# COMBINE-lab/RapMap

Measured on AMD Instinct MI355X. Metric: Mreads/s (paired 2x100 bp; one unit = one read pair), higher is better.
Workload: dtype u8/int32/u64 (integer & byte work, no floating point)

## Files before the change

### rapmap_amd/csrc/qm_host.hip

```cpp
#include <fcntl.h>
#include <hip/hip_runtime.h>
#include <sys/mman.h>
#include <sys/stat.h>
#include <unistd.h>

#include <atomic>
#include <cmath>
#include <cstdarg>
#include <cstdio>
#include <cstdlib>
#include <cstring>
#include <deque>
#include <string>
#include <vector>
#include <thread>
#include <map>
#include <memory>
#include <mutex>
#include <condition_variable>
#include <functional>

#include "qm_mapper.inl"
#include "qm_lean.inl"
#include "qm_device.h"
#include "qm_phflat.h"

using namespace qm;

static thread_local char g_err[512] = "";
static int fail(int code, const char* fmt, ...) {
  va_list ap; va_start(ap, fmt); vsnprintf(g_err, sizeof(g_err), fmt, ap); va_end(ap);
  return code;
}
#define HIPCHK(x) do { hipError_t _e = (x); if (_e != hipSuccess) return fail(QM_E_NOGPU, "%s: %s", #x, hipGetErrorString(_e)); } while (0)

struct MMap {
  void* p = nullptr; size_t len = 0;
  int open(const std::string& path) {
    int fd = ::open(path.c_str(), O_RDONLY);
    if (fd < 0) return -1;
    struct stat st; if (fstat(fd, &st) != 0) { ::close(fd); return -1; }
    len = (size_t)st.st_size;
    if (len == 0) { ::close(fd); return -1; }
    p = mmap(nullptr, len, PROT_READ, MAP_PRIVATE, fd, 0);
    ::close(fd);
    if (p == MAP_FAILED) { p = nullptr; return -1; }
    return 0;
  }
  void close() { if (p) munmap(p, len); p = nullptr; }
};

struct qm_index {
  std::string dir;
  int k = 31; bool big = false, perfect = false;
  MMap sa, txp, rsd, hash;
  const uint32_t* SA = nullptr; int64_t nSA = 0;
  std::vector<std::string> names;
  const uint32_t* offsets = nullptr; int64_t nTxp = 0;
// ... 130 lines not shown
  DevBuf<long long> d_toff;
  DevBuf<qm_hit> d_tmp; DevBuf<unsigned char> d_sides; DevBuf<int> d_tsc;
  DevBuf<int> d_tref; DevBuf<u64> d_torder; DevBuf<unsigned char> d_tasks;
  DevBuf<long long> d_ivcsr, d_lcsr;
  DevBuf<qm_sa_interval_hit> d_ivC; DevBuf<u64> d_wordsC;
  PinBuf<long long> h_tot;
  LastResult last; CallStats stats;
  uint32_t flags = 0; bool isHelper = false;
  std::vector<qm_ctx*> helpers; struct SplitPool* pool = nullptr;
};

struct SplitPool {
  std::vector<std::thread> th; std::mutex mu; std::condition_variable cv, done;
  std::function<void(int)> job; unsigned long gen = 0; int pending = 0, parts = 0; bool stop = false;
  explicit SplitPool(int n) {
    for (int i = 0; i < n; ++i) th.emplace_back([this, i]() {
      unsigned long seen = 0;
      for (;;) {
        std::function<void(int)> j;
        { std::unique_lock<std::mutex> lk(mu); cv.wait(lk, [&] { return stop || (gen != seen && i < parts); }); if (stop) return; seen = gen; j = job; }
        j(i);
        { std::lock_guard<std::mutex> lk(mu); if (--pending == 0) done.notify_all(); }
      }
    });
  }
  void run(int n, std::function<void(int)> f) {
    std::unique_lock<std::mutex> lk(mu);
    job = std::move(f); parts = n; pending = n; ++gen;
    cv.notify_all();
    done.wait(lk, [&] { return pending == 0; });
  }
  ~SplitPool() { { std::lock_guard<std::mutex> lk(mu); stop = true; } cv.notify_all(); for (auto& t : th) t.join(); }
};
struct SplitJoin {
  qm_ctx* owner; int K; std::mutex mu; std::condition_variable cv;
  long long total[8] = {0}, base[9] = {0}; int arrived = 0; bool ready = false; int failed = 0;
  int arrive(int part, long long tot, long long& b, qm_hit*& dst);
  void abort(int rc) { std::lock_guard<std::mutex> lk(mu); if (!failed) failed = rc ? rc : QM_E_STATE; cv.notify_all(); }
  bool stagger = false; int turn = 0;
  int wait_turn(int part) {
    if (!stagger) return QM_OK;
    std::unique_lock<std::mutex> lk(mu);
    cv.wait(lk, [&] { return turn >= part || failed; });
    return failed ? fail(failed, "another part of the batch failed") : QM_OK;
  }
  void pass_turn(int part) { if (!stagger) return; std::lock_guard<std::mutex> lk(mu); if (turn < part + 1) turn = part + 1; cv.notify_all(); }
};

static void begin_call(qm_ctx* c) { c->last.invalidate(); c->stats = CallStats(); }

extern "C" {

const char* qm_last_error(void) { return g_err; }
const char* qm_version(void) { return "qmap_mi355 0.1 (RapMap 0.6.0 quasimap hot path, gfx950)"; }

int qm_opts_default(qm_opts* o) {
  if (!o) return fail(QM_E_ARG, "null opts");
  o->sensitive = 1; o->strict_check = 1; o->max_num_hits = 200; o->no_orphans = 0; o->no_dovetail = 0;
  o->fuzzy = 0; o->max_interval = 1000; o->sel_aln = 0; o->quasi_cov = 0.0;
  o->hard_filter = 0; o->match_score = 2; o->mismatch_penalty = -4; o->gap_open = 4; o->gap_extend = 2; o->dp_bandwidth = 15;
  o->max_mmp_extension = 7; o->aln_policy = 0; o->min_score_fraction = 0.65; o->consensus_slack = 0.2;
  return QM_OK;
}

static bool json_field(const std::string& js, const char* name, std::string& out) {
  std::string key = std::string("\"") + name + "\"";
  size_t p = js.find(key);
  if (p == std::string::npos) return false;
  p = js.find(':', p);
  if (p == std::string::npos) return false;
  ++p;
// ... 738 lines not shown

enum { QM_STAGE_RETRY = 1 };
static int stage_verdict(qm_ctx* c, const StagePlan& p, const u64* hscal) {
  const int status = (int)(hscal[QM_SC_STATUS] & 0xffffffffu); int rc;
  if (status & 4) return fail(QM_E_TOOLONG, "a read is longer than %d characters (-s: the alignment kernels are sized for that; otherwise the long-read pass takes up to %d)", QM_MAX_LONG_READ_LEN, QM_MAX_LONG_READ_LEN);
  if (status & 2) return fail(QM_E_UNSUPPORTED, "an SA-interval list exceeded %d entries (max_interval too large)", QM_GCAP);
  if (status & 8) return fail(QM_E_STATE, "selective alignment: a read overflowed the scratch sized for it (internal error)");
  if (status & 64) return fail(QM_E_STATE, "a wavefront found no free scratch slot on its XCD (internal error)");
  if (!(status & 17)) return QM_OK;
  if (status & 1) {
    int64_t want = (int64_t)hscal[0] + p.nreads + (int64_t)p.grid * 4 * QM_CHUNK;
    if (want < c->d_lists.cap * 2) want = c->d_lists.cap * 2;
    if ((rc = c->d_lists.ensure(want))) return rc;
  }
  if (status & 16) {
    int64_t want = (int64_t)hscal[QM_SC_IVCUR] + p.nreads + (int64_t)p.grid * 4 * QM_IVCHUNK;
    if (want < c->d_iv.cap * 2) want = c->d_iv.cap * 2;
    if ((rc = c->d_iv.ensure(want))) return rc;
  }
  c->stats.relaunches += 1;
  return QM_STAGE_RETRY;
}

static int run_stage_a(qm_ctx* c, const qm_opts* o, const RunReq& rq, int64_t n, const void* d_seq1, const void* d_off1, const void* d_seq2,
                       const void* d_off2, int ns, ChunkFeeder* feeder, u64* hscal) {
  int rc; StagePlan p;
  if ((rc = plan_stage_a(c, o, rq, d_seq2 != nullptr, n, ns, p))) return rc;
  if ((rc = reserve_stage_a(c, o, rq, p))) return rc;
  const DevIndex ix = dev_index(c);
  const int64_t nreads = p.nreads;
  if (lean_first(p)) c->stats.leanReads = nreads;
  if (p.first == SK_DUO) c->stats.duoPairs = n;
  float extraMs = 0;
  while (true) {
    ReadBatch B;
    fill_batch(c, o, rq, p, d_seq1, d_off1, d_seq2, d_off2, B);
    ReadBatch H = B;
    if (p.twoPass) { H.iv_in = c->d_iv; H.iv_in_off = c->d_ivoff; H.iv_in_cnt = c->d_ivcnt; H.found_in = c->d_found; H.iv_out = nullptr; H.found_out = nullptr; }
    HIPCHK(hipMemsetAsync(c->d_scal, 0, QM_SC_WORDS * sizeof(u64), c->stream));
    if (rq.mode == QM_RUN_COLLECT || p.twoPass) HIPCHK(hipMemsetAsync(c->d_lcnt, 0, (size_t)(nreads + 1) * sizeof(uint32_t), c->stream));
    HIPCHK(hipEventRecord(c->ev0, c->stream));
    if ((rc = launch_first(c, p, rq, ix, B, feeder))) return rc;
    feeder = nullptr;
    if (p.first == SK_LEAN_SEL && nreads > 0) {
      if ((rc = read_scalars(c, hscal)) || (rc = pass_n_aware(c, p, ix, B, hscal, extraMs)) || (rc = pass_lean_leftovers(c, p, ix, B, hscal, extraMs))) return rc;
      c->stats.leanReads = nreads;
    }
    if (p.twoPass && rq.longReads && nreads > 0 && ((rc = read_scalars(c, hscal)) || (rc = pass_long_reads(c, p, ix, B, hscal, -32)))) return rc;
    if ((rc = run_list_kernels(c, p, rq, ix, H))) return rc;
    HIPCHK(hipEventRecord(c->ev1, c->stream));
    if ((rc = read_scalars(c, hscal))) return rc;
    if (lean_first(p) && ((rc = pass_n_aware(c, p, ix, B, hscal, extraMs)) || (rc = pass_lean_leftovers(c, p, ix, B, hscal, extraMs)))) return rc;
    if ((!o->sel_aln || rq.mode == QM_RUN_COLLECT) && rq.mode != QM_RUN_FROM_INTERVALS && (rc = pass_long_reads(c, p, ix, B, hscal, rq.mode == QM_RUN_COLLECT ? -32 : 32))) return rc;
    if ((rc = pass_sel_slow(c, o, rq, ix, H, hscal))) return rc;
#ifdef QM_TIMING
    {
      static const char* nm[7] = {"read->LDS", "strand setup", "probe windows", "extension", "collector rest", "hits->mappings", "write-out+loop"};
      double tot = 0; for (int i = 0; i < 7; ++i) tot += (double)hscal[20 + i];
      for (int i = 0; i < 7; ++i) fprintf(stderr, "[qm timing] %-16s %6.2f %%  %10.0f clk/read\n", nm[i], 100.0 * hscal[20 + i] / tot, (double)hscal[20 + i] / (double)nreads);
      static const char* hm[8] = {"intervals in", "suffix gather", "sort", "groups+chain", "list assembly", "(after)", "write-out", "-"};
      double ht = 0; for (int i = 0; i < 8; ++i) ht += (double)hscal[32 + i];
      if (ht > 0) for (int i = 0; i < 8; ++i) fprintf(stderr, "[qm timing h2m] %-16s %6.2f %%  %10.0f clk/read\n", hm[i], 100.0 * hscal[32 + i] / ht, (double)hscal[32 + i] / (double)nreads);
      static const char* pm[8] = {"cand+intervals", "gather+keys", "rank sort", "heads+count", "chaining", "words", "write-out", "chaining, parallel"};
      double pt = 0; for (int i = 0; i < 8; ++i) pt += (double)hscal[40 + i];
      if (pt > 0) for (int i = 0; i < 8; ++i) fprintf(stderr, "[qm timing pack] %-16s %6.2f %%  %10.0f clk/read\n", pm[i], 100.0 * hscal[40 + i] / pt, (double)hscal[40 + i] / (double)nreads);
    }
#endif
    if ((rc = stage_verdict(c, p, hscal)) == QM_STAGE_RETRY) continue;
    if (rc) return rc;
    break;
  }
  c->stats.skipped = (int64_t)hscal[QM_SC_SKIPCNT];
  if (c->stats.skipped > 0) {
    c->stats.skipList.resize((size_t)(c->stats.skipped < QM_SKIP_CAP ? c->stats.skipped : QM_SKIP_CAP));
    HIPCHK(hipMemcpy(c->stats.skipList.data(), c->d_skip, c->stats.skipList.size() * sizeof(u64), hipMemcpyDeviceToHost));
  }
  if (p.wantIv) { c->last.ivTotal = (int64_t)hscal[QM_SC_IVCUR]; c->last.ivReads = nreads; }
  if (p.wantFound) c->last.foundReads = nreads;
  if (rq.mode != QM_RUN_COLLECT && !p.duoMerge) c->last.listReads = nreads;
  c->last.listWords = (int64_t)hscal[0];
  float ms = 0; hipEventElapsedTime(&ms, c->ev0, c->ev1); c->last.mapMs = ms + extraMs;
  return QM_OK;
}
// ... 69 lines not shown
      for (int i = 0; i < K; ++i) {
        Ak[i] = A; Ak[i].u0 = cu[i]; Ak[i].u1 = cu[i + 1];
        Ak[i].tasks = (SelTask*)(c->d_tasks + (size_t)(2 * cslot[i] + 2 * i) * qmk_sel_task_bytes());
        Ak[i].ntasks = c->d_ntk + i;
        Ak[i].sides = (SelSide*)(c->d_sides + (size_t)(2 * cslot[i] + 2 * i) * qmk_sel_side_bytes());
        Ak[i].nsides = c->d_ntk + QM_SEL_CHUNKS_B + i;
        Ak[i].torder = c->d_torder + (size_t)(2 * cslot[i] + 2 * i);
        if (!noStrip) { Ak[i].torder2 = c->d_torder + (size_t)(2 * slots + 2 * K + 2) + (size_t)(2 * cslot[i] + 2 * i); Ak[i].ntasks2 = c->d_ntk + 2 * QM_SEL_CHUNKS_B + i; }
        HIPCHK(qmk_sel_plan(&P, &Ak[i], c->numCU, planStream));
        if (K > 1) HIPCHK(hipEventRecord(c->evPlan[i], planStream));
      }
      for (int i = 0; i < K; ++i) {
        if (K > 1) HIPCHK(hipStreamWaitEvent(c->stream, c->evPlan[i], 0));
        HIPCHK(qmk_sel_align_finish(&P, &Ak[i], c->numCU, c->stream));
      }
    }
  } else {
    HIPCHK(qmk_pair_count(&P, c->stream));
  }
  HIPCHK(qmk_scan_counts(c->d_scanTmp, (size_t)c->d_scanTmp.cap, c->d_cnt, c->d_offs, n + 1, c->stream));
  total = 0;
  HIPCHK(hipMemcpyAsync(&total, c->d_offs + n, sizeof(long long), hipMemcpyDeviceToHost, c->stream));
  HIPCHK(hipMemcpyAsync(hscal, c->d_scal, QM_SC_WORDS * sizeof(u64), hipMemcpyDeviceToHost, c->stream));
  u64 h[3 * QM_SEL_CHUNKS_B];
  const bool selStats = o->sel_aln && !rq.mergeOnly;
  if (selStats) HIPCHK(hipMemcpyAsync(h, c->d_ntk, sizeof(h), hipMemcpyDeviceToHost, c->stream));
  HIPCHK(hipStreamSynchronize(c->stream));
  if (selStats) {
    for (int i = 0; i < QM_SEL_CHUNKS_B; ++i) { c->stats.kswTasks += (int64_t)h[i]; c->stats.selQuestions += (int64_t)h[QM_SEL_CHUNKS_B + i]; c->stats.stripTasks += (int64_t)h[2 * QM_SEL_CHUNKS_B + i]; }
    static const bool dbg = [] { const char* e = getenv("QM_SEL_DEBUG"); return e && atoi(e) != 0; }();
    if (dbg) fprintf(stderr, "[qm -s] %lld units: %lld alignment questions beyond PERFECT chains, %lld ksw2 alignments, %lld strip alignments\n", (long long)n, (long long)c->stats.selQuestions, (long long)c->stats.kswTasks, (long long)c->stats.stripTasks);
  }
  if (rq.join) {
    long long b = 0; qm_hit* dst = nullptr;
    if ((rc = rq.join->arrive(rq.part, total, b, dst))) return rc;
    P.hits = dst + b;
  } else {
    if ((rc = c->d_hits.ensure((int64_t)total + 1, total / 8))) return rc;
    P.hits = c->d_hits;
  }
  if (o->sel_aln) HIPCHK(qmk_sel_compact(&P, c->d_tmp, c->d_toff, c->stream));
  else HIPCHK(qmk_pair_write(&P, c->stream));
  return QM_OK;
}

static int map_device_impl(qm_ctx* c, const qm_opts* o, int64_t n, const void* d_seq1, const void* d_off1, const void* d_seq2,
                           const void* d_off2, int32_t max_read_len, int64_t* n_hits, qm_counters* counters, ChunkFeeder* feeder,
                           const RunReq& rq = RunReq(), int32_t short_read_len = 0) {
  if (!c || n < 0 || (n > 0 && (!d_seq1 || !d_off1))) return fail(QM_E_ARG, "bad argument");
  int rc = check_opts(o);
  if (rc) return rc;
  if ((d_seq2 == nullptr) != (d_off2 == nullptr)) return fail(QM_E_ARG, "seq2/off2 must both be given or both be null");
  HIPCHK(hipSetDevice(c->device));
  const int pick = (max_read_len > QM_MAX_READ_LEN && short_read_len > 0) ? short_read_len : (max_read_len > QM_MAX_READ_LEN ? QM_MAX_READ_LEN : max_read_len);
  const int ns = pick <= 128 ? 2 : (pick <= 192 ? 3 : (pick <= 256 ? 4 : 8));
  const bool paired = d_seq2 != nullptr;
  u64 hscal[QM_SC_WORDS];
  begin_call(c);
  HIPCHK(hipEventRecord(c->evA, c->stream));
  RunReq r2 = rq;
  r2.keepIntervals = rq.keepIntervals || c->debug != 0;
  r2.longReads = max_read_len > QM_MAX_READ_LEN;
  r2.shortLen = pick;
  if (rq.join && (rc = rq.join->wait_turn(rq.part))) return rc;
  rc = run_stage_a(c, o, r2, n, d_seq1, d_off1, d_seq2, d_off2, ns, feeder, hscal);
  if (rq.join) rq.join->pass_turn(rq.part);
  if (rc) return rc;
  if (r2.stageView) {
    const int64_t nreads = paired ? 2 * n : n;
    if ((rc = c->d_ivcsr.ensure(nreads + 1))) return rc;
    if ((rc = c->d_lcsr.ensure(nreads + 1))) return rc;
    if ((rc = c->h_tot.ensure(2))) return rc;
    if ((rc = ensure_scan_tmp(c, nreads + 1))) return rc;
    if (!r2.keepIntervals) {
      if ((rc = c->d_ivcnt.ensure(nreads + 1))) return rc;
      if ((rc = c->d_ivoff.ensure(nreads + 1))) return rc;
      if ((rc = c->d_iv.ensure(1))) return rc;
      HIPCHK(hipMemsetAsync(c->d_ivcnt, 0, (size_t)(nreads + 1) * sizeof(uint32_t), c->stream));
      HIPCHK(hipMemsetAsync(c->d_ivoff, 0, (size_t)(nreads + 1) * sizeof(long long), c->stream));
    }
    HIPCHK(hipMemsetAsync(c->d_ivcnt + nreads, 0, sizeof(uint32_t), c->stream));
    HIPCHK(hipMemsetAsync(c->d_lcnt + nreads, 0, sizeof(uint32_t), c->stream));
    HIPCHK(qmk_scan_counts(c->d_scanTmp, (size_t)c->d_scanTmp.cap, c->d_ivcnt, c->d_ivcsr, nreads + 1, c->stream));
    HIPCHK(qmk_scan_counts_masked(c->d_scanTmp, (size_t)c->d_scanTmp.cap, c->d_lcnt, c->d_lcsr, nreads + 1, c->stream));
    HIPCHK(hipMemcpyAsync(&c->h_tot[0], c->d_ivcsr + nreads, sizeof(long long), hipMemcpyDeviceToHost, c->stream));
    HIPCHK(hipMemcpyAsync(&c->h_tot[1], c->d_lcsr + nreads, sizeof(long long), hipMemcpyDeviceToHost, c->stream));
    c->last.stReads = nreads;
  }
  long long total = 0;
  if ((rc = run_stage_b(c, o, r2, n, paired, d_seq1, d_off1, d_seq2, d_off2, hscal, total))) return rc;
  HIPCHK(hipEventRecord(c->evB, c->stream));
  HIPCHK(hipStreamSynchronize(c->stream));
  float ms = 0; hipEventElapsedTime(&ms, c->evA, c->evB); c->last.totalMs = ms;
  c->last.units = n; c->last.hits = total; c->last.paired = paired;
  if (r2.stageView) c->last.stUnits = n;
  if (n_hits) *n_hits = total;
  if (counters) *counters = counters_from(hscal);
  return QM_OK;
}

int SplitJoin::arrive(int part, long long tot, long long& b, qm_hit*& dst) {
  std::unique_lock<std::mutex> lk(mu);
  total[part] = tot;
  if (++arrived == K && !failed) {
    for (int i = 0; i < K; ++i) base[i + 1] = base[i] + total[i];
    const int rc = owner->d_hits.ensure((int64_t)base[K] + 1, base[K] / 8);
    if (rc) failed = rc; else ready = true;
    cv.notify_all();
  }
  cv.wait(lk, [&] { return ready || failed; });
  if (failed) return failed == QM_E_NOMEM ? fail(QM_E_NOMEM, "hipMalloc of the result array failed") : fail(failed, "another part of the batch failed");
  b = base[part]; dst = owner->d_hits;
  return QM_OK;
}

static int map_device_split(qm_ctx* c, const qm_opts* o, int K, int64_t n, const void* d_seq1, const void* d_off1, const void* d_seq2,
                            const void* d_off2, int32_t max_read_len, int64_t* n_hits, qm_counters* counters) {
  int rc;
  HIPCHK(hipSetDevice(c->device));
  while ((int)c->helpers.size() < K) {
    qm_ctx* h = nullptr;
    if ((rc = qm_ctx_create_ex(c->ix, c->device, c->flags, &h))) return rc;
    h->isHelper = true; c->helpers.push_back(h);
  }
  if (!c->pool || (int)c->pool->th.size() < K) { delete c->pool; c->pool = new SplitPool(K); }
  if ((rc = c->d_offs.ensure(n + 1))) return rc;
  SplitJoin J; J.owner = c; J.K = K;
  { const char* sg = getenv("QM_SPLIT_STAGGER"); J.stagger = sg ? atoi(sg) != 0 : false; }
  int64_t nh[8] = {0}; qm_counters ctr[8]; int rcs[8] = {0}; char errs[8][256];
  memset(ctr, 0, sizeof(ctr));
  const bool paired = d_seq2 != nullptr;
  static const int firstPct = [] { const char* e = getenv("QM_SPLIT_FIRST"); const int v = e ? atoi(e) : 0; return v > 0 && v < 100 ? v : 0; }();
  static const int duoParts = [] { const char* e = getenv("QM_DUO_PARTS"); return e ? atoi(e) : 0x55; }();
  begin_call(c);
  HIPCHK(hipEventRecord(c->evA, c->stream));
  c->pool->run(K, [&](int i) {
    qm_ctx* h = c->helpers[(size_t)i];
    int64_t u0 = n * i / K, u1 = n * (i + 1) / K;
    if (K == 2 && firstPct > 0) { const int64_t cut = n * firstPct / 100; u0 = i == 0 ? 0 : cut; u1 = i == 0 ? cut : n; }
    RunReq rq; rq.join = &J; rq.part = i;
    rq.noDuo = ((duoParts >> i) & 1) == 0;
    errs[i][0] = 0;
    int r = map_device_impl(h, o, u1 - u0, d_seq1, (const long long*)d_off1 + u0, d_seq2, d_seq2 ? (const long long*)d_off2 + u0 : nullptr,
                            max_read_len, &nh[i], &ctr[i], nullptr, rq);
    if (r == QM_OK) {
      hipError_t e = qmk_rebase_offsets(h->d_offs, c->d_offs + u0, (u1 - u0) + (i == K - 1 ? 1 : 0), J.base[i], h->stream);
      if (e == hipSuccess) e = hipStreamSynchronize(h->stream);
      if (e != hipSuccess) r = fail(QM_E_NOGPU, "rebasing a part's offsets: %s", hipGetErrorString(e));
    }
    if (r != QM_OK) { snprintf(errs[i], sizeof(errs[i]), "%s", g_err); J.abort(r); }
    rcs[i] = r;
  });
  for (int i = 0; i < K; ++i) if (rcs[i]) return fail(rcs[i], "%s", errs[i]);
  HIPCHK(hipEventRecord(c->evB, c->stream));
  HIPCHK(hipEventSynchronize(c->evB));
  float first = 1e30f, last = 0, t = 0;
  for (int i = 0; i < K; ++i) {
    qm_ctx* h = c->helpers[(size_t)i];
    if (hipEventElapsedTime(&t, c->evA, h->ev0) == hipSuccess && t < first) first = t;
    if (hipEventElapsedTime(&t, c->evA, h->ev1) == hipSuccess && t > last) last = t;
  }
  c->last.mapMs = last > first ? last - first : 0;
  float ms = 0; hipEventElapsedTime(&ms, c->evA, c->evB); c->last.totalMs = ms;
  qm_counters sum; memset(&sum, 0, sizeof(sum));
  for (int i = 0; i < K; ++i) {
    sum += ctr[i];
    int64_t u0 = n * i / K;
    if (K == 2 && firstPct > 0) u0 = i == 0 ? 0 : n * firstPct / 100;
    c->stats.add_part(c->helpers[(size_t)i]->stats, paired ? 2 * u0 : u0);
  }
  c->last.units = n; c->last.hits = J.base[K]; c->last.paired = paired;
  if (n_hits) *n_hits = J.base[K];
  if (counters) *counters = sum;
  return QM_OK;
}

int qm_map_device(qm_ctx* c, const qm_opts* o, int64_t n, const void* d_seq1, const void* d_off1, const void* d_seq2,
                  const void* d_off2, int32_t max_read_len, int64_t* n_hits, qm_counters* counters) {
  const char* me = getenv("QM_SPLIT_MIN");
  const int64_t minUnits = me && atoll(me) > 0 ? atoll(me) : ((int64_t)1 << 21);
  if (c && o && !c->isHelper && !c->debug && n >= minUnits && d_seq1 && d_off1 && (d_seq2 == nullptr) == (d_off2 == nullptr) && check_opts(o) == QM_OK) {
    const char* se = getenv("QM_SPLIT");
    int K = se ? atoi(se) : 2;
    if (K > 8) K = 8;
    if (K > 1) return map_device_split(c, o, K, n, d_seq1, d_off1, d_seq2, d_off2, max_read_len, n_hits, counters);
  }
  return map_device_impl(c, o, n, d_seq1, d_off1, d_seq2, d_off2, max_read_len, n_hits, counters, nullptr);
}

static int stage_offsets(qm_ctx* c, int64_t n, const int64_t* off, DevBuf<uint8_t>& d_seq, DevBuf<long long>& d_off, int32_t& maxLen,
                         int32_t& maxShort) {
  for (int64_t i = 0; i < n; ++i) {
    int64_t l = off[i + 1] - off[i];
    if (l < 0) return fail(QM_E_ARG, "offsets not monotone");
    if (l > maxLen) maxLen = (int32_t)(l > 0x7fffffff ? 0x7fffffff : l);
    if (l <= QM_MAX_READ_LEN && l > maxShort) maxShort = (int32_t)l;
  }
  int rc;
  if ((rc = d_seq.ensure(off[n] + 64))) return rc;
  if ((rc = d_off.ensure(n + 1))) return rc;
  HIPCHK(hipMemcpyAsync(d_off, off, (size_t)(n + 1) * 8, hipMemcpyHostToDevice, c->copyStream));
  return QM_OK;
}

struct HostFeed { qm_ctx* c; const char* seq1; const int64_t* off1; const char* seq2; const int64_t* off2; };
static int host_feed_upload(void* self, int64_t u0, int64_t u1) {
  HostFeed* f = (HostFeed*)self;
  const int64_t a1 = f->off1[u0], b1 = f->off1[u1];
  if (b1 > a1) HIPCHK(hipMemcpyAsync(f->c->d_seq1 + a1, f->seq1 + a1, (size_t)(b1 - a1), hipMemcpyHostToDevice, f->c->copyStream));
  if (f->seq2) {
    const int64_t a2 = f->off2[u0], b2 = f->off2[u1];
    if (b2 > a2) HIPCHK(hipMemcpyAsync(f->c->d_seq2 + a2, f->seq2 + a2, (size_t)(b2 - a2), hipMemcpyHostToDevice, f->c->copyStream));
  }
  return QM_OK;
}

static int map_host(qm_ctx* c, const qm_opts* o, int64_t n, const char* seq1, const int64_t* off1, const char* seq2,
                    const int64_t* off2, int64_t* n_hits, qm_counters* counters, const RunReq& rq) {
// ... 462 lines not shown
```

### rapmap_amd/csrc/qm_kernels.hip

```cpp
#include <hip/hip_runtime.h>
#include <cstring>
#include <type_traits>
#include <cstdlib>
#include <rocprim/rocprim.hpp>

#include "qm_mapper.inl"
#include "qm_device.h"

namespace qm {

#ifndef QM_H2M_WPS
#define QM_H2M_WPS 4
#endif
template <int F>
__global__ __launch_bounds__(256, QM_H2M_WPS) void qm_h2m_kernel(DevIndex ix, ReadBatch B) {
  __shared__ H2mMem mem[4];
  __shared__ SelLds<(F & QM_F_SEL) != 0> sels[4];
  const int wave = __builtin_amdgcn_readfirstlane((int)(threadIdx.x >> 6));
  const long long gw = (long long)blockIdx.x * 4 + wave;
  qm_tim_begin(wave);
  h2m_wave<F>(ix, B, gw, (long long)gridDim.x * 4, mem[wave], B.gscratch + gw * QM_GSCR_U64, (F & QM_F_SEL) ? B.selscr + gw : nullptr, sels[wave].ptr(),
              ((F & QM_F_SEL) && B.dyn) ? B.dyn + gw : nullptr);
  qm_tim_flush(B.cursor, wave, 32, 8);
}
// ... 11 lines not shown

__global__ __launch_bounds__(256, 2) void qm_h2m_packw_kernel(DevIndex ix, ReadBatch B, const long long* ids, const u64* nids, long long* todoq) {
  __shared__ PackMemW<4> mem[4];
  const int wave = __builtin_amdgcn_readfirstlane((int)(threadIdx.x >> 6));
  qm_tim_begin(wave);
  packw_wave<4>(ix, B, ids, nids, (long long)blockIdx.x * 4 + wave, (long long)gridDim.x * 4, mem[wave], todoq);
  qm_tim_flush(B.cursor, wave, 40, 8);
}

__global__ __launch_bounds__(256) void qm_pair_count_kernel(PairBatch P) {
  __shared__ unsigned long long sc[6];
  if (threadIdx.x < 6) sc[threadIdx.x] = 0;
  __syncthreads();
  long long u = (long long)blockIdx.x * blockDim.x + threadIdx.x;
  UnitCounters uc = {0, 0, 0, 0, 0, 0};
  if (u < P.n) P.cnt[u] = (u32)unit_merge(P, u, nullptr, 0, &uc);
  if (uc.pe) atomicAdd(&sc[0], uc.pe);
  if (uc.se) atomicAdd(&sc[1], uc.se);
  if (uc.tot) atomicAdd(&sc[2], uc.tot);
  if (uc.reads) atomicAdd(&sc[3], uc.reads);
  if (uc.tooMany) atomicAdd(&sc[4], uc.tooMany);
  if (uc.mapped) atomicAdd(&sc[5], uc.mapped);
  __syncthreads();
  if (threadIdx.x < 6 && sc[threadIdx.x]) atomicAdd((unsigned long long*)&P.counters[threadIdx.x], sc[threadIdx.x]);
}

#define QM_PW_CAP 320
static_assert(sizeof(qm_hit) == 32, "the staged write passes (qm_pair_write_kernel, qm_sel_compact_kernel) copy a hit as two uint4");
__global__ __launch_bounds__(256) void qm_pair_write_kernel(PairBatch P) {
  __shared__ __attribute__((aligned(16))) qm_hit stage[4][QM_PW_CAP];
  const int wave = __builtin_amdgcn_readfirstlane((int)(threadIdx.x >> 6)), lane = (int)(threadIdx.x & 63u);
  const long long u = (long long)blockIdx.x * blockDim.x + threadIdx.x;
  const int c = u < P.n ? (int)P.cnt[u] : 0;
  int incl = c;
  for (int d = 1; d < 64; d <<= 1) { const int t = __shfl_up(incl, d); if (lane >= d) incl += t; }
  const int total = __shfl(incl, 63);
  if (total == 0) return;
  if (total > QM_PW_CAP) {
    if (c > 0) unit_merge(P, u, P.hits + P.offs[u], c, nullptr);
    return;
  }
  if (c > 0) unit_merge(P, u, &stage[wave][incl - c], c, nullptr);
  const long long base = __shfl(c > 0 ? P.offs[u] - (long long)(incl - c) : 0LL, __builtin_ctzll(__ballot(c > 0)));
  __builtin_amdgcn_fence(__ATOMIC_SEQ_CST, "workgroup");
  __builtin_amdgcn_wave_barrier();
  const uint4* src = (const uint4*)&stage[wave][0];
  uint4* dst = (uint4*)(P.hits + base);
  for (int i = lane; i < 2 * total; i += 64) dst[i] = src[i];
}

__global__ __launch_bounds__(256) void qm_sel_slots_kernel(PairBatch P) {
  long long u = (long long)blockIdx.x * blockDim.x + threadIdx.x;
  if (u > P.n) return;
  u32 w = 0;
  if (u < P.n) w = P.paired ? (P.lcnt[2 * u] & 0x7fffffffu) + (P.lcnt[2 * u + 1] & 0x7fffffffu) : (P.lcnt[u] & 0x7fffffffu);
  P.cnt[u] = u < P.n ? w / 3 + 1 : 0;
}

QM_DEV void sel_flush_counters(unsigned long long* sc, const UnitCounters& uc, u64* counters) {
  if (uc.pe) atomicAdd(&sc[0], uc.pe);
  if (uc.se) atomicAdd(&sc[1], uc.se);
  if (uc.tot) atomicAdd(&sc[2], uc.tot);
  if (uc.reads) atomicAdd(&sc[3], uc.reads);
  if (uc.tooMany) atomicAdd(&sc[4], uc.tooMany);
  if (uc.mapped) atomicAdd(&sc[5], uc.mapped);
  __syncthreads();
// ... 642 lines not shown
  } else
  switch (sel_ksw_ring_slots(A.bandwidth)) {
    case 32:
      if (A.short_len > 0 && A.short_len <= 128) hipLaunchKernelGGL(qm_sel_align2_kernel<128 + 32>, dim3((unsigned)(num_cu * 8 * ao)), dim3(256), 0, st, P, A);
      else if (A.short_len > 0 && A.short_len <= 192) hipLaunchKernelGGL(qm_sel_align2_kernel<192 + 32>, dim3((unsigned)(num_cu * 8 * ao)), dim3(256), 0, st, P, A);
      else if (A.short_len > 0 && A.short_len <= 256) hipLaunchKernelGGL(qm_sel_align2_kernel<256 + 32>, dim3((unsigned)(num_cu * 7 * ao)), dim3(256), 0, st, P, A);
      else hipLaunchKernelGGL(qm_sel_align2_kernel<QM_KSW_MAXLEN>, dim3((unsigned)(num_cu * 4 * ao)), dim3(256), 0, st, P, A);
      break;
    case 64: hipLaunchKernelGGL((qm_sel_align_kernel<64, 4>), dim3((unsigned)(num_cu * 8 * ao)), dim3(256), 0, st, P, A); break;
    case 128: hipLaunchKernelGGL((qm_sel_align_kernel<128, 4>), dim3((unsigned)(num_cu * 4 * ao)), dim3(256), 0, st, P, A); break;
    default: hipLaunchKernelGGL((qm_sel_align_kernel<1024, 2>), dim3((unsigned)(num_cu * 2 * ao)), dim3(128), 0, st, P, A); break;
  }
  hipLaunchKernelGGL(qm_sel_finish_kernel, dim3(nb), dim3(256), 0, st, P, A);
  return hipGetLastError();
}
size_t qmk_sel_task_bytes(void) { return sizeof(SelTask); }
size_t qmk_sel_gmem_rows_bytes(int num_cu) { return (size_t)num_cu * QMK_GMEM_WAVES * 4 * sizeof(KswRowT<QM_KSW_RING_GMEM, QM_KSW_MAXLEN_LONG>); }
hipError_t qmk_sel_compact(const void* pp, const void* tmp, const void* toff, hipStream_t st) {
  const PairBatch& P = *(const PairBatch*)pp;
  if (P.n <= 0) return hipSuccess;
  hipLaunchKernelGGL(qm_sel_compact_kernel, dim3((unsigned)((P.n + 255) / 256)), dim3(256), 0, st, P, (const qm_hit*)tmp, (const long long*)toff);
  return hipGetLastError();
}

hipError_t qmk_pair_count(const void* pp, hipStream_t st) {
  const PairBatch& P = *(const PairBatch*)pp;
  if (P.n <= 0) return hipSuccess;
  hipLaunchKernelGGL(qm_pair_count_kernel, dim3((unsigned)((P.n + 255) / 256)), dim3(256), 0, st, P);
  return hipGetLastError();
}

hipError_t qmk_pair_write(const void* pp, hipStream_t st) {
  const PairBatch& P = *(const PairBatch*)pp;
  if (P.n <= 0) return hipSuccess;
  hipLaunchKernelGGL(qm_pair_write_kernel, dim3((unsigned)((P.n + 255) / 256)), dim3(256), 0, st, P);
  return hipGetLastError();
}

hipError_t qmk_unpack_reads(const unsigned char* packed, const long long* off, long long n, long long total_chars, unsigned char* seq, const void* exc,
                            long long n_exc, hipStream_t st) {
  if (n > 0) {
    const long long threads = n * (long long)QM_UNPACK_TPR;
    hipLaunchKernelGGL(qm_unpack_kernel, dim3((unsigned)((threads + 255) / 256)), dim3(256), 0, st, packed, off, n, seq);
  }
  if (n_exc > 0) hipLaunchKernelGGL(qm_unpack_exc_kernel, dim3((unsigned)((n_exc + 255) / 256)), dim3(256), 0, st, (const qm_pack_exc*)exc, n_exc, seq, (unsigned long long)total_chars);
  return hipGetLastError();
}

size_t qmk_scan_temp_bytes(long long n) {
  size_t bytes = 0;
  auto it = rocprim::make_transform_iterator((const u32*)nullptr, U32ToI64());
  (void)rocprim::exclusive_scan(nullptr, bytes, it, (long long*)nullptr, 0LL, (size_t)n, rocprim::plus<long long>());
  return bytes;
}

hipError_t qmk_scan_counts(void* temp, size_t temp_bytes, const u32* cnt, long long* offs, long long n, hipStream_t st) {
  auto it = rocprim::make_transform_iterator(cnt, U32ToI64());
  return rocprim::exclusive_scan(temp, temp_bytes, it, offs, 0LL, (size_t)n, rocprim::plus<long long>(), st);
}

hipError_t qmk_scan_counts_masked(void* temp, size_t temp_bytes, const u32* cnt, long long* offs, long long n, hipStream_t st) {
  auto it = rocprim::make_transform_iterator(cnt, U32MaskToI64());
  return rocprim::exclusive_scan(temp, temp_bytes, it, offs, 0LL, (size_t)n, rocprim::plus<long long>(), st);
}

hipError_t qmk_stage_gather(long long nreads, const u32* ivcnt, const long long* ivoff, const void* iv, const long long* ivcsr, void* iv_out,
                            const u32* lcnt, const long long* loff, const unsigned long long* lists, const long long* lcsr,
                            unsigned long long* words_out, hipStream_t st) {
// ... 8 lines not shown
```

Measured before the change: 482.8.

## Let split parts write hits early, fold offset rebasing into the write kernel, add chained waves

Replaces the split-batch join with a ledger. When all earlier parts have arrived and the result buffer is large enough, a part can start its write-out right away, instead of every part waiting for the full total. If the buffer must grow later, the early writers are synchronized and the write is redone. The pair-write kernel now also stores rebased offsets, which removes the separate rebase launch and its stream sync in the non-alignment path. An optional multi-wave split chains each stage A after the stage A of the part two places earlier via events, but its default wave count of 1 leaves it off. It also adds profiling scripts.

After: 481.4, median of 2. No clear change (-0.3%).

```diff
diff --git a/profiles/split_waves/figures.py b/profiles/split_waves/figures.py
--- /dev/null
+++ b/profiles/split_waves/figures.py
@@ -0,0 +1,12 @@
+#!/usr/bin/env python3
+import json
+import sys
+
+label = sys.argv[1]
+line = [l for l in sys.stdin.read().splitlines() if l.startswith("{")]
+if not line:
+    print("%-22s no result line" % label)
+    sys.exit(1)
+j = json.loads(line[-1])
+ms, k = j["ms_per_step"], j["config"]["map_kernel_ms"]
+print("%-22s M pairs/s %8.3f  ms_per_step %7.3f  map_kernel_ms %7.3f  gap %6.3f  hits_per_pair %.4f" % (label, j["value"], ms, k, ms - k, j["config"]["hits_per_pair"]))
diff --git a/profiles/split_waves/timeline.py b/profiles/split_waves/timeline.py
--- /dev/null
+++ b/profiles/split_waves/timeline.py
@@ -0,0 +1,28 @@
+#!/usr/bin/env python3
+import csv
+import glob
+import sys
+
+d, parts = sys.argv[1], int(sys.argv[2])
+f = glob.glob(d + "/**/*kernel_trace.csv", recursive=True)[0]
+rows = sorted(csv.DictReader(open(f)), key=lambda r: int(r["Start_Timestamp"]))
+name = lambda r: r["Kernel_Name"].split("(")[0].replace("void ", "")[:70]
+dur = lambda r: (int(r["End_Timestamp"]) - int(r["Start_Timestamp"])) / 1e6
+stage_a = [i for i, r in enumerate(rows) if ("qm_lean_kernel" in r["Kernel_Name"] or "qm_duo_kernel" in r["Kernel_Name"]) and dur(r) > 1.0]
+last = stage_a[-parts:]
+t0 = int(rows[last[0]]["Start_Timestamp"])
+ms = lambda t: (int(t) - t0) / 1e6
+print("# the last step of the run; start_ms end_ms dur_ms queue kernel")
+for r in rows[last[0]:]:
+    print("%9.3f %9.3f %8.3f  q%-3s %s" % (ms(r["Start_Timestamp"]), ms(r["End_Timestamp"]), dur(r), r.get("Queue_Id", "?"), name(r)))
+a_end = max(ms(rows[i]["End_Timestamp"]) for i in last)
+end = max(ms(r["End_Timestamp"]) for r in rows[last[0]:])
+print("# stage A: first start 0.000, last end %.3f; last kernel of the step ends %.3f: %.3f ms behind stage A" % (a_end, end, end - a_end))
+for kind in ("qm_duo_kernel", "qm_lean_kernel"):
+    iv = sorted((ms(rows[i]["Start_Timestamp"]), ms(rows[i]["End_Timestamp"])) for i in last if kind in rows[i]["Kernel_Name"])
+    gaps = ["%.3f" % (b[0] - a[1]) for a, b in zip(iv, iv[1:])]
+    print("# %s: %s; gaps between consecutive launches (ms): %s" % (kind, " ".join("[%.3f, %.3f]" % x for x in iv), " ".join(gaps) or "-"))
+for kind in ("qm_duo_kernel", "qm_lean_kernel"):
+    ds = [dur(rows[i]) for i in stage_a if kind in rows[i]["Kernel_Name"]]
+    per_step = [sum(ds[j:j + parts // 2]) for j in range(0, len(ds) - parts // 2 + 1, parts // 2)]
+    print("# %s: %d launches; sum of the launches of a step, ms: %s" % (kind, len(ds), " ".join("%.3f" % x for x in per_step)))
diff --git a/rapmap_amd/csrc/qm_host.hip b/rapmap_amd/csrc/qm_host.hip
--- a/rapmap_amd/csrc/qm_host.hip
+++ b/rapmap_amd/csrc/qm_host.hip
@@ -24,6 +24,7 @@
 #include "qm_lean.inl"
 #include "qm_device.h"
 #include "qm_phflat.h"
+#include "qm_split.h"
 
 using namespace qm;
 
@@ -220,11 +221,12 @@
   }
   ~SplitPool() { { std::lock_guard<std::mutex> lk(mu); stop = true; } cv.notify_all(); for (auto& t : th) t.join(); }
 };
-struct SplitJoin {
-  qm_ctx* owner; int K; std::mutex mu; std::condition_variable cv;
-  long long total[8] = {0}, base[9] = {0}; int arrived = 0; bool ready = false; int failed = 0;
-  int arrive(int part, long long tot, long long& b, qm_hit*& dst);
-  void abort(int rc) { std::lock_guard<std::mutex> lk(mu); if (!failed) failed = rc ? rc : QM_E_STATE; cv.notify_all(); }
+struct SplitJoin : SplitLedger {
+  qm_ctx* owner = nullptr; int64_t u[QM_SPLIT_MAX_PARTS + 1] = {0};
+  bool chained = false;
+  int arrive(int part, long long tot, const std::function<int(long long)>& write);
+  int chain_stage_a(int part, hipStream_t st);
+  void stage_a_ended(int part) { if (chained) stage_a_recorded(part); }
   bool stagger = false; int turn = 0;
   int wait_turn(int part) {
     if (!stagger) return QM_OK;
@@ -1029,6 +1031,7 @@
   if (lean_first(p)) c->stats.leanReads = nreads;
   if (p.first == SK_DUO) c->stats.duoPairs = n;
   float extraMs = 0;
+  if (rq.join && (rc = rq.join->chain_stage_a(rq.part, c->stream))) return rc;
   while (true) {
     ReadBatch B;
     fill_batch(c, o, rq, p, d_seq1, d_off1, d_seq2, d_off2, B);
@@ -1046,6 +1049,7 @@
     if (p.twoPass && rq.longReads && nreads > 0 && ((rc = read_scalars(c, hscal)) || (rc = pass_long_reads(c, p, ix, B, hscal, -32)))) return rc;
     if ((rc = run_list_kernels(c, p, rq, ix, H))) return rc;
     HIPCHK(hipEventRecord(c->ev1, c->stream));
+    if (rq.join) rq.join->stage_a_ended(rq.part);
     if ((rc = read_scalars(c, hscal))) return rc;
     if (lean_first(p) && ((rc = pass_n_aware(c, p, ix, B, hscal, extraMs)) || (rc = pass_lean_leftovers(c, p, ix, B, hscal, extraMs)))) return rc;
     if ((!o->sel_aln || rq.mode == QM_RUN_COLLECT) && rq.mode != QM_RUN_FROM_INTERVALS && (rc = pass_long_reads(c, p, ix, B, hscal, rq.mode == QM_RUN_COLLECT ? -32 : 32))) return rc;
@@ -1181,13 +1185,17 @@
     if (dbg) fprintf(stderr, "[qm -s] %lld units: %lld alignment questions beyond PERFECT chains, %lld ksw2 alignments, %lld strip alignments\n", (long long)n, (long long)c->stats.selQuestions, (long long)c->stats.kswTasks, (long long)c->stats.stripTasks);
   }
   if (rq.join) {
-    long long b = 0; qm_hit* dst = nullptr;
-    if ((rc = rq.join->arrive(rq.part, total, b, dst))) return rc;
-    P.hits = dst + b;
-  } else {
-    if ((rc = c->d_hits.ensure((int64_t)total + 1, total / 8))) return rc;
-    P.hits = c->d_hits;
-  }
+    SplitJoin& J = *rq.join;
+    return J.arrive(rq.part, total, [&](long long b) -> int {
+      P.hits = J.owner->d_hits + b;
+      if (o->sel_aln) { HIPCHK(qmk_sel_compact(&P, c->d_tmp, c->d_toff, c->stream)); return QM_OK; }
+      P.offs_out = J.owner->d_offs + J.u[rq.part]; P.offs_add = b; P.offs_close = rq.part == J.K - 1 ? 1 : 0;
+      HIPCHK(qmk_pair_write(&P, c->stream));
+      return QM_OK;
+    });
+  }
+  if ((rc = c->d_hits.ensure((int64_t)total + 1, total / 8))) return rc;
+  P.hits = c->d_hits;
   if (o->sel_aln) HIPCHK(qmk_sel_compact(&P, c->d_tmp, c->d_toff, c->stream));
   else HIPCHK(qmk_pair_write(&P, c->stream));
   return QM_OK;
@@ -1248,24 +1256,23 @@
   return QM_OK;
 }
 
-int SplitJoin::arrive(int part, long long tot, long long& b, qm_hit*& dst) {
-  std::unique_lock<std::mutex> lk(mu);
-  total[part] = tot;
-  if (++arrived == K && !failed) {
-    for (int i = 0; i < K; ++i) base[i + 1] = base[i] + total[i];
-    const int rc = owner->d_hits.ensure((int64_t)base[K] + 1, base[K] / 8);
-    if (rc) failed = rc; else ready = true;
-    cv.notify_all();
-  }
-  cv.wait(lk, [&] { return ready || failed; });
-  if (failed) return failed == QM_E_NOMEM ? fail(QM_E_NOMEM, "hipMalloc of the result array failed") : fail(failed, "another part of the batch failed");
-  b = base[part]; dst = owner->d_hits;
-  return QM_OK;
-}
-
-static int map_device_split(qm_ctx* c, const qm_opts* o, int K, int64_t n, const void* d_seq1, const void* d_off1, const void* d_seq2,
-                            const void* d_off2, int32_t max_read_len, int64_t* n_hits, qm_counters* counters) {
-  int rc;
+int SplitJoin::arrive(int part, long long tot, const std::function<int(long long)>& write) {
+  g_err[0] = 0;
+  const int rc = join(part, tot, write);
+  if (rc && !g_err[0]) return rc == QM_E_NOMEM ? fail(QM_E_NOMEM, "hipMalloc of the result array failed") : fail(rc, "another part of the batch failed");
+  return rc;
+}
+int SplitJoin::chain_stage_a(int part, hipStream_t st) {
+  if (!chained || part < 2) return QM_OK;
+  const int rc = wait_stage_a_recorded(part - 2);
+  if (rc) return fail(rc, "another part of the batch failed");
+  HIPCHK(hipStreamWaitEvent(st, owner->helpers[(size_t)(part - 2)]->ev1, 0));
+  return QM_OK;
+}
+
+static int map_device_split(qm_ctx* c, const qm_opts* o, int K, const int64_t* u, bool chained, const void* d_seq1, const void* d_off1,
+                            const void* d_seq2, const void* d_off2, int32_t max_read_len, int64_t* n_hits, qm_counters* counters) {
+  int rc; const int64_t n = u[K];
   HIPCHK(hipSetDevice(c->device));
   while ((int)c->helpers.size() < K) {
     qm_ctx* h = nullptr;
@@ -1274,25 +1281,27 @@
   }
   if (!c->pool || (int)c->pool->th.size() < K) { delete c->pool; c->pool = new SplitPool(K); }
   if ((rc = c->d_offs.ensure(n + 1))) return rc;
-  SplitJoin J; J.owner = c; J.K = K;
+  SplitJoin J; J.owner = c; J.K = K; J.chained = chained;
+  for (int i = 0; i <= K; ++i) J.u[i] = u[i];
+  J.cap = c->d_hits.cap; J.early = !o->sel_aln;
+  J.grow = [c](long long need, long long& cap) -> int { const int r = c->d_hits.ensure((int64_t)need, (need - 1) / 8); cap = c->d_hits.cap; return r; };
+  J.sync_writer = [c](int part) -> int { HIPCHK(hipStreamSynchronize(c->helpers[(size_t)part]->stream)); return QM_OK; };
   { const char* sg = getenv("QM_SPLIT_STAGGER"); J.stagger = sg ? atoi(sg) != 0 : false; }
   int64_t nh[8] = {0}; qm_counters ctr[8]; int rcs[8] = {0}; char errs[8][256];
   memset(ctr, 0, sizeof(ctr));
   const bool paired = d_seq2 != nullptr;
-  static const int firstPct = [] { const char* e = getenv("QM_SPLIT_FIRST"); const int v = e ? atoi(e) : 0; return v > 0 && v < 100 ? v : 0; }();
   static const int duoParts = [] { const char* e = getenv("QM_DUO_PARTS"); return e ? atoi(e) : 0x55; }();
   begin_call(c);
   HIPCHK(hipEventRecord(c->evA, c->stream));
   c->pool->run(K, [&](int i) {
     qm_ctx* h = c->helpers[(size_t)i];
-    int64_t u0 = n * i / K, u1 = n * (i + 1) / K;
-    if (K == 2 && firstPct > 0) { const int64_t cut = n * firstPct / 100; u0 = i == 0 ? 0 : cut; u1 = i == 0 ? cut : n; }
+    const int64_t u0 = u[i], u1 = u[i + 1];
     RunReq rq; rq.join = &J; rq.part = i;
     rq.noDuo = ((duoParts >> i) & 1) == 0;
     errs[i][0] = 0;
     int r = map_device_impl(h, o, u1 - u0, d_seq1, (const long long*)d_off1 + u0, d_seq2, d_seq2 ? (const long long*)d_off2 + u0 : nullptr,
                             max_read_len, &nh[i], &ctr[i], nullptr, rq);
-    if (r == QM_OK) {
+    if (r == QM_OK && o->sel_aln) {
       hipError_t e = qmk_rebase_offsets(h->d_offs, c->d_offs + u0, (u1 - u0) + (i == K - 1 ? 1 : 0), J.base[i], h->stream);
       if (e == hipSuccess) e = hipStreamSynchronize(h->stream);
       if (e != hipSuccess) r = fail(QM_E_NOGPU, "rebasing a part's offsets: %s", hipGetErrorString(e));
@@ -1314,9 +1323,7 @@
   qm_counters sum; memset(&sum, 0, sizeof(sum));
   for (int i = 0; i < K; ++i) {
     sum += ctr[i];
-    int64_t u0 = n * i / K;
-    if (K == 2 && firstPct > 0) u0 = i == 0 ? 0 : n * firstPct / 100;
-    c->stats.add_part(c->helpers[(size_t)i]->stats, paired ? 2 * u0 : u0);
+    c->stats.add_part(c->helpers[(size_t)i]->stats, paired ? 2 * u[i] : u[i]);
   }
   c->last.units = n; c->last.hits = J.base[K]; c->last.paired = paired;
   if (n_hits) *n_hits = J.base[K];
@@ -1331,8 +1338,20 @@
   if (c && o && !c->isHelper && !c->debug && n >= minUnits && d_seq1 && d_off1 && (d_seq2 == nullptr) == (d_off2 == nullptr) && check_opts(o) == QM_OK) {
     const char* se = getenv("QM_SPLIT");
     int K = se ? atoi(se) : 2;
-    if (K > 8) K = 8;
-    if (K > 1) return map_device_split(c, o, K, n, d_seq1, d_off1, d_seq2, d_off2, max_read_len, n_hits, counters);
+    if (K > QM_SPLIT_MAX_PARTS) K = QM_SPLIT_MAX_PARTS;
+    const char* we = getenv("QM_SPLIT_WAVES"); const char* pe = getenv("QM_SPLIT_LAST_PCT");
+    const int W = we ? atoi(we) : QM_SPLIT_WAVES_DEFAULT, pct = pe ? atoi(pe) : QM_SPLIT_LAST_PCT_DEFAULT;
+    int64_t u[QM_SPLIT_MAX_PARTS + 1];
+    if (!se && !o->sel_aln && W > 1) {
+      K = qm_split_wave_bounds(n, W, pct, u);
+      return map_device_split(c, o, K, u, K > 2, d_seq1, d_off1, d_seq2, d_off2, max_read_len, n_hits, counters);
+    }
+    if (K > 1) {
+      static const int firstPct = [] { const char* e = getenv("QM_SPLIT_FIRST"); const int v = e ? atoi(e) : 0; return v > 0 && v < 100 ? v : 0; }();
+      qm_split_even_bounds(n, K, u);
+      if (K == 2 && firstPct > 0) u[1] = n * firstPct / 100;
+      return map_device_split(c, o, K, u, false, d_seq1, d_off1, d_seq2, d_off2, max_read_len, n_hits, counters);
+    }
   }
   return map_device_impl(c, o, n, d_seq1, d_off1, d_seq2, d_off2, max_read_len, n_hits, counters, nullptr);
 }
diff --git a/rapmap_amd/csrc/qm_kernels.hip b/rapmap_amd/csrc/qm_kernels.hip
--- a/rapmap_amd/csrc/qm_kernels.hip
+++ b/rapmap_amd/csrc/qm_kernels.hip
@@ -67,6 +67,7 @@
   const int wave = __builtin_amdgcn_readfirstlane((int)(threadIdx.x >> 6)), lane = (int)(threadIdx.x & 63u);
   const long long u = (long long)blockIdx.x * blockDim.x + threadIdx.x;
   const int c = u < P.n ? (int)P.cnt[u] : 0;
+  if (P.offs_out && (u < P.n || (u == P.n && P.offs_close))) P.offs_out[u] = P.offs[u] + P.offs_add;
   int incl = c;
   for (int d = 1; d < 64; d <<= 1) { const int t = __shfl_up(incl, d); if (lane >= d) incl += t; }
   const int total = __shfl(incl, 63);
@@ -775,8 +776,9 @@
 
 hipError_t qmk_pair_write(const void* pp, hipStream_t st) {
   const PairBatch& P = *(const PairBatch*)pp;
-  if (P.n <= 0) return hipSuccess;
-  hipLaunchKernelGGL(qm_pair_write_kernel, dim3((unsigned)((P.n + 255) / 256)), dim3(256), 0, st, P);
+  const long long threads = P.n + (P.offs_out && P.offs_close ? 1 : 0);
+  if (threads <= 0) return hipSuccess;
+  hipLaunchKernelGGL(qm_pair_write_kernel, dim3((unsigned)((threads + 255) / 256)), dim3(256), 0, st, P);
   return hipGetLastError();
 }
 
diff --git a/rapmap_amd/csrc/qm_split.h b/rapmap_amd/csrc/qm_split.h
--- /dev/null
+++ b/rapmap_amd/csrc/qm_split.h
@@ -0,0 +1,85 @@
+#pragma once
+#include <condition_variable>
+#include <cstdint>
+#include <functional>
+#include <mutex>
+
+#define QM_SPLIT_MAX_PARTS 8
+#define QM_SPLIT_WAVES_DEFAULT 1
+#define QM_SPLIT_LAST_PCT_DEFAULT 20
+
+static inline int qm_split_wave_bounds(int64_t n, int W, int lastPct, int64_t* u) {
+  if (W > QM_SPLIT_MAX_PARTS / 2) W = QM_SPLIT_MAX_PARTS / 2;
+  if (lastPct < 1) lastPct = 1;
+  if (lastPct > 99) lastPct = 99;
+  for (; W > 1; --W) {
+    const int64_t last = n * lastPct / 100, rest = n - last;
+    bool ok = last >= 2;
+    int64_t w[QM_SPLIT_MAX_PARTS / 2 + 1];
+    for (int j = 0; j < W; ++j) w[j] = rest * j / (W - 1);
+    w[W] = n;
+    for (int j = 0; j < W; ++j) ok = ok && w[j + 1] - w[j] >= 2;
+    if (!ok) continue;
+    for (int j = 0; j < W; ++j) { u[2 * j] = w[j]; u[2 * j + 1] = w[j] + (w[j + 1] - w[j]) / 2; }
+    u[2 * W] = n;
+    return 2 * W;
+  }
+  u[0] = 0; u[1] = n / 2; u[2] = n;
+  return 2;
+}
+static inline void qm_split_even_bounds(int64_t n, int K, int64_t* u) { for (int i = 0; i <= K; ++i) u[i] = n * i / K; }
+
+struct SplitLedger {
+  int K = 0;
+  long long cap = 0;
+  bool early = true;
+  std::function<int(long long need, long long& newCap)> grow;
+  std::function<int(int part)> sync_writer;
+  std::mutex mu; std::condition_variable cv;
+  long long total[QM_SPLIT_MAX_PARTS] = {0}, base[QM_SPLIT_MAX_PARTS + 1] = {0};
+  bool here[QM_SPLIT_MAX_PARTS] = {false}, wrote[QM_SPLIT_MAX_PARTS] = {false}, stageAEnd[QM_SPLIT_MAX_PARTS] = {false};
+  int arrived = 0, failed = 0, growths = 0; bool done = false, grown = false;
+
+  bool prefix_here(int part) {
+    for (int i = 0; i < part; ++i) if (!here[i]) return false;
+    long long b = 0;
+    for (int i = 0; i < part; ++i) b += total[i];
+    base[part] = b;
+    return true;
+  }
+  int join(int part, long long tot, const std::function<int(long long)>& write) {
+    std::unique_lock<std::mutex> lk(mu);
+    total[part] = tot; here[part] = true;
+    if (++arrived == K && !failed) {
+      for (int i = 0; i < K; ++i) base[i + 1] = base[i] + total[i];
+      if (base[K] + 1 > cap) {
+        int rc = 0;
+        for (int i = 0; i < K && !rc; ++i) if (wrote[i]) rc = sync_writer(i);
+        long long nc = cap;
+        if (!rc) rc = grow(base[K] + 1, nc);
+        if (rc) failed = rc; else { cap = nc; grown = true; ++growths; }
+      }
+      done = true;
+    }
+    cv.notify_all();
+    cv.wait(lk, [&] { return failed || done || (early && prefix_here(part) && base[part] + tot + 1 <= cap); });
+    if (failed) return failed;
+    if (!done) {
+      int rc = write(base[part]);
+      if (rc) return rc;
+      wrote[part] = true;
+      cv.wait(lk, [&] { return failed || done; });
+      if (failed) return failed;
+      if (!grown) return 0;
+    }
+    return write(base[part]);
+  }
+  void abort(int rc) { std::lock_guard<std::mutex> lk(mu); if (!failed) failed = rc ? rc : -1; cv.notify_all(); }
+
+  void stage_a_recorded(int part) { std::lock_guard<std::mutex> lk(mu); stageAEnd[part] = true; cv.notify_all(); }
+  int wait_stage_a_recorded(int part) {
+    std::unique_lock<std::mutex> lk(mu);
+    cv.wait(lk, [&] { return stageAEnd[part] || failed; });
+    return failed;
+  }
+};
```
